# acids-ircam/RAVE

Hardware: NVIDIA H100
Metric: audio-seconds/s (v2 train step fwd+bwd, 48 kHz) (higher is better)
Workload: dtype bf16

## Files before the change

include/rave_b200.h:

```cpp
#ifndef RAVE_B200_H
#define RAVE_B200_H

#include <stddef.h>
#include <stdint.h>

#ifdef __cplusplus
extern "C" {
#endif

#define RAVE_ACT_NONE 0
#define RAVE_ACT_LEAKY 1
#define RAVE_ACT_SNAKE 2

#define RAVE_PREC_FP32 0
#define RAVE_PREC_BF16 1
#define RAVE_PREC_TF32 2

int rave_b200_version(void);
const char *rave_b200_last_error(void);
unsigned long long rave_b200_launch_count(void);

int rave_pqmf_analysis_fwd(const float *x, const float *taps, float *y, int B, int T, int Lout,
                           int ntaps, int pad_l, int flip_sign, void *stream);
int rave_pqmf_synthesis_fwd(const float *x, const float *w, float *out, int B, int L, int K,
                            int pad_l, float scale, int flip_sign, void *stream);
int rave_pqmf_analysis_fast(const float *x, const float *Ct, const float *Qt, float *y, int B, int T, int Lout,
                            int pad_l, int flip_sign, void *stream);
int rave_pqmf_synthesis_fast(const float *x, const float *Cc, const float *Qt, float *out, int B, int L,
                             int pad_l, float scale, int flip_sign, void *stream);

int rave_conv1d_gather_f32(const float *src, const float *w, const float *bias, const float *res,
                           float *out, int B, int Cs, int Ls, int Cm, int Lo, int K, int stride,
                           int dil, int pad_l, long ws_m, long ws_c, int act, float slope,
                           const float *alpha, int post_act, float post_slope, const float *post_x,
                           const float *post_alpha, void *stream);
int rave_conv1d_scatter_f32(const float *src, const float *w, const float *bias, const float *res,
                            float *out, int B, int Cs, int Ls, int Cm, int Lo, int K, int stride,
                            int dil, int pad_l, long ws_m, long ws_c, int act, float slope,
                            const float *alpha, int post_act, float post_slope, const float *post_x,
                            const float *post_alpha, void *stream);

size_t rave_conv1d_wgrad_workspace_bytes(int B, int Ca, int Cc, int Lp, int K);
int rave_conv1d_wgrad_f32(const float *P, const float *Q, float *dw, int B, int Ca, int Lp, int Cc,
                          int Lq, int K, int stride, int dil, int pad_l, long os_a, long os_c,
                          int act_p, int act_q, float slope, const float *alpha, void *workspace,
                          void *stream);

int rave_weight_norm_fwd(const float *v, const float *g, float *w, float *norm_out, int C0, int R,
                         void *stream);
int rave_weight_norm_bwd(const float *dw, const float *v, const float *g, const float *norm,
                         float *dv, float *dg, int C0, int R, void *stream);

int rave_act_fwd(const float *x, float *y, int B, int C, int L, int act, float slope,
                 const float *alpha, void *stream);
int rave_act_bwd(const float *dy, const float *x, float *dx, float *dalpha, int B, int C, int L,
                 int act, float slope, const float *alpha, void *stream);
int rave_am_tanh_fwd(const float *x, float *y, int B, int C, int L, void *stream);
int rave_am_tanh_bwd(const float *dy, const float *x, float *dx, int B, int C, int L, void *stream);
int rave_reparam_fwd(const float *z, const float *eps, float *zs, float *kl_sum, int B, int C, int L, void *stream);
int rave_mmd_fwd(const float *z, const float *prior, float *means, float *mmd, int B, int D, int L, void *stream);
int rave_mmd_bwd(const float *z, const float *prior, const float *g, float *dz, int B, int D, int L, void *stream);
int rave_sphere_norm_fwd(const float *z, float *out, float *norm, int B, int C, int L, void *stream);
int rave_sphere_norm_bwd(const float *g, const float *out, const float *norm, float *dz, int B, int C, int L,
                         void *stream);

int rave_conv1d_tc_supported(int Cin, int Cout, int K, int stride, int dil);
int rave_dilated_unit_tc_supported(int C, int L);
int rave_dilated_unit_tc_fwd(const void *xa_bf16, const void *w3t_bf16, const void *w1t_bf16, void *a1_out,
                             float *out_f32, void *out_act, int B, int C, int L, int pitch, int dil, int pad_l,
                             float slope_in, float slope_mid, int act_out, float slope_out, void *stream);
int rave_conv1d_tc_plan(int B, int Cin, int Cout, int Lout, int K);
int rave_conv1d_tc_pp_stages(int B, int Cin, int Cout, int Lout, int K, int fm, int res_bf16);
int rave_conv1d_tc_fwd(const void *xa_bf16, const void *wt_bf16, const float *bias, const float *res,
                       const void *res_bf16, const void *dact_src_bf16, const void *res_act_bf16, float res_slope,
                       float *out_f32, void *out_act_bf16,
                       int B, int Cin, int Lin, int in_pitch, int Cout, int Lout,
                       int K, int stride, int dil, int pad_l, int act, float slope, int out_rows,
                       int out_row_stride, int out_row_offset, const float *fm_d, int fm_bh, void *stream);
int rave_conv1d_tc_fwd_x3(const void *xa_bf16, const void *wt_bf16, const float *bias, const float *res,
                          const void *res_act, float res_slope, float *out_f32, void *out_act, int B, int Cin, int Lin,
                          int in_pitch, int Cout, int Lout, int K, int stride, int dil, int pad_l, int act, float slope,
                          int out_rows, int out_row_stride, int out_row_offset, int act_cs, void *stream);
int rave_conv1d_tc_wgrad_splits(int B, int Cm, int Lp, int Cn, int K);
int rave_time_stack_cl(const float *x, void *out_bf16, int B, int C, int T, int F, int Fp, int Cp, int kt, int pt,
                       void *stream);
int rave_time_stack_cl_bwd(const void *g_bf16, float *gx, int B, int C, int T, int F, int Fp, int Cp, int kt, int pt,
                           void *stream);
int rave_time_stack_nhwc(const float *x, void *out_bf16, int B, int C, int T, int F, long sb, long st, int Fp, int Cp, int kt,
                         int pt, void *stream);
int rave_time_stack_nhwc_bwd(const void *g_bf16, float *gx, int B, int C, int T, int F, int Fp, int Cp, int kt, int pt,
                             void *stream);
int rave_time_stack_nhwc_dil(const float *x, void *out_bf16, int B, int C, int T, int F, long sb, long st, int Fp, int Cp,
                             int kt, int pt, int dil, void *stream);
int rave_time_stack_nhwc_dil_bwd(const void *g_bf16, float *gx, int B, int C, int T, int F, int Fp, int Cp, int kt, int pt,
                                 int dil, void *stream);
int rave_l1_stats_f32(const float *t, const float *v, float *stats, long n, void *stream);
int rave_l1_grad_f32(const float *t, const float *v, const float *d, float *gt, float *gv, long n, void *stream);
int rave_leaky_fm_fwd(const float *x, float *a, float *stats, long H, float slope, void *stream);
int rave_leaky_fm_bwd(const float *a, const float *g, const float *d, float *gx, long H, float slope, void *stream);
int rave_leaky_fm_stack_fwd(const float *x, float *a, float *stats, void *xs_bf16, long Rh, int T, int F, int C, int Fp,
                            float slope, void *stream);
int rave_leaky_fm_stack_bwd(const float *a, const void *gxs_bf16, const float *ga, const float *d, float *gx, long Rh, int T,
                            int F, int C, int Fp, float slope, void *stream);
int rave_leaky_fm_stack_dil_fwd(const float *x, float *a, float *stats, void *xs_bf16, long Rh, int T, int F, int C, int Fp,
                                int dil, float slope, void *stream);
int rave_leaky_fm_stack_dil_bwd(const float *a, const void *gxs_bf16, const float *ga, const float *d, float *gx, long Rh,
                                int T, int F, int C, int Fp, int dil, float slope, void *stream);
int rave_snake_cl_fwd(const void *h_bf16, const float *alpha, void *a_bf16, long rows, int C, void *stream);
int rave_snake_cl_bwd(const void *ga_bf16, const void *h_bf16, const float *alpha, const void *add_bf16, void *gh_bf16,
                      float *dalpha, long rows, int C, void *stream);
int rave_conv1d_tc_wgrad(const void *P_bf16, const void *Q_bf16, float *dwt, float *dbias, int B, int Cm, int Lp,
                         int p_pitch, int Cn, int Lq, int q_pitch, int K, int stride, int dil, int pad_l,
                         void *stream);
int rave_tapmajor_to_weight_f32(const float *dwt, float *dw, int Cm, int Cn, int K, int transpose, int splits,
                                void *stream);
int rave_conv1d_c1_fwd(const float *x, const float *w, const float *bias, float *out_f32, void *out_act_bf16,
                       int R, int x_pitch, int Lin, int Cout, int Lout, int out_pitch, int K, int stride,
                       int pad_l, int act, float slope, void *stream);
int rave_conv1d_c1_wgrad_splits(int R, int Lout);
int rave_conv1d_c1_wgrad(const void *g_bf16, const float *x, float *dwt, int R, int x_pitch, int Lin, int Cout,
                         int Cg, int Lout, int g_pitch, int K, int stride, int pad_l, void *stream);
int rave_conv1d_c1_dgrad(const void *g_bf16, const float *w, float *dx, int R, int x_pitch, int Lin, int Cout,
                         int Cg, int Lout, int g_pitch, int K, int stride, int pad_l, void *stream);
int rave_colsum_bf16(const void *g_bf16, float *out, int R, int L, int pitch, int Cg, int C, void *stream);
int rave_im2col_c1(const float *src, void *X_bf16, int R, int src_pitch, int src_len, int Lin, int Lout,
// ... 79 lines not shown
```

rave_b200/_lib.py:

```python
import ctypes
import os
from ctypes import c_float, c_int, c_long, c_size_t, c_ulonglong, c_void_p, c_char_p

_HERE = os.path.dirname(os.path.abspath(__file__))
LIB_PATH = os.path.join(_HERE, "csrc", "librave_b200.so")

_P, _I, _F, _L = c_void_p, c_int, c_float, c_long

SIGNATURES = {
    "rave_b200_version": (c_int, []),
    "rave_b200_last_error": (c_char_p, []),
    "rave_b200_launch_count": (c_ulonglong, []),
    "rave_pqmf_analysis_fwd": (c_int, [_P, _P, _P, _I, _I, _I, _I, _I, _I, _P]),
    "rave_pqmf_synthesis_fwd": (c_int, [_P, _P, _P, _I, _I, _I, _I, _F, _I, _P]),
    "rave_pqmf_analysis_fast": (c_int, [_P, _P, _P, _P, _I, _I, _I, _I, _I, _P]),
    "rave_pqmf_synthesis_fast": (c_int, [_P, _P, _P, _P, _I, _I, _I, _F, _I, _P]),
    "rave_conv1d_gather_f32": (c_int, [_P, _P, _P, _P, _P, _I, _I, _I, _I, _I, _I, _I, _I, _I, _L, _L,
                                       _I, _F, _P, _I, _F, _P, _P, _P]),
    "rave_conv1d_scatter_f32": (c_int, [_P, _P, _P, _P, _P, _I, _I, _I, _I, _I, _I, _I, _I, _I, _L, _L,
                                        _I, _F, _P, _I, _F, _P, _P, _P]),
    "rave_conv1d_wgrad_workspace_bytes": (c_size_t, [_I, _I, _I, _I, _I]),
    "rave_conv1d_wgrad_f32": (c_int, [_P, _P, _P, _I, _I, _I, _I, _I, _I, _I, _I, _I, _L, _L, _I, _I,
                                      _F, _P, _P, _P]),
    "rave_weight_norm_fwd": (c_int, [_P, _P, _P, _P, _I, _I, _P]),
    "rave_weight_norm_bwd": (c_int, [_P, _P, _P, _P, _P, _P, _I, _I, _P]),
    "rave_act_fwd": (c_int, [_P, _P, _I, _I, _I, _I, _F, _P, _P]),
    "rave_act_bwd": (c_int, [_P, _P, _P, _P, _I, _I, _I, _I, _F, _P, _P]),
    "rave_am_tanh_fwd": (c_int, [_P, _P, _I, _I, _I, _P]),
    "rave_am_tanh_bwd": (c_int, [_P, _P, _P, _I, _I, _I, _P]),
    "rave_reparam_fwd": (c_int, [_P, _P, _P, _P, _I, _I, _I, _P]),
    "rave_mmd_fwd": (c_int, [_P, _P, _P, _P, _I, _I, _I, _P]),
    "rave_mmd_bwd": (c_int, [_P, _P, _P, _P, _I, _I, _I, _P]),
    "rave_sphere_norm_fwd": (c_int, [_P, _P, _P, _I, _I, _I, _P]),
    "rave_sphere_norm_bwd": (c_int, [_P, _P, _P, _P, _I, _I, _I, _P]),
    "rave_conv1d_tc_supported": (c_int, [_I, _I, _I, _I, _I]),
    "rave_dilated_unit_tc_supported": (c_int, [_I, _I]),
    "rave_dilated_unit_tc_fwd": (c_int, [_P, _P, _P, _P, _P, _P, _I, _I, _I, _I, _I, _I, _F, _F, _I, _F, _P]),
    "rave_conv1d_tc_plan": (c_int, [_I, _I, _I, _I, _I]),
    "rave_conv1d_tc_pp_stages": (c_int, [_I, _I, _I, _I, _I, _I, _I]),
    "rave_conv1d_tc_fwd": (c_int, [_P, _P, _P, _P, _P, _P, _P, _F, _P, _P, _I, _I, _I, _I, _I, _I, _I, _I, _I, _I, _I,
                                   _F, _I, _I, _I, _P, _I, _P]),
    "rave_conv1d_tc_fwd_x3": (c_int, [_P, _P, _P, _P, _P, _F, _P, _P, _I, _I, _I, _I, _I, _I, _I, _I, _I, _I, _I, _F, _I,
                                      _I, _I, _I, _P]),
    "rave_weight_prep_tc_multi_x3": (c_int, [_I, _P, _P]),
    "rave_ncl_to_cl_x3": (c_int, [_P, _P, _I, _I, _I, _P]),
    "rave_conv1d_tc_wgrad": (c_int, [_P, _P, _P, _P, _I, _I, _I, _I, _I, _I, _I, _I, _I, _I, _I, _P]),
    "rave_tapmajor_to_weight_f32": (c_int, [_P, _P, _I, _I, _I, _I, _I, _P]),
    "rave_conv1d_tc_wgrad_splits": (c_int, [_I, _I, _I, _I, _I]),
    "rave_time_stack_cl": (c_int, [_P, _P, _I, _I, _I, _I, _I, _I, _I, _I, _P]),
    "rave_time_stack_cl_bwd": (c_int, [_P, _P, _I, _I, _I, _I, _I, _I, _I, _I, _P]),
    "rave_time_stack_nhwc": (c_int, [_P, _P, _I, _I, _I, _I, ctypes.c_long, ctypes.c_long, _I, _I, _I, _I, _P]),
    "rave_time_stack_nhwc_bwd": (c_int, [_P, _P, _I, _I, _I, _I, _I, _I, _I, _I, _P]),
    "rave_time_stack_nhwc_dil": (c_int, [_P, _P, _I, _I, _I, _I, ctypes.c_long, ctypes.c_long, _I, _I, _I, _I, _I, _P]),
    "rave_time_stack_nhwc_dil_bwd": (c_int, [_P, _P, _I, _I, _I, _I, _I, _I, _I, _I, _I, _P]),
    "rave_l1_stats_f32": (c_int, [_P, _P, _P, ctypes.c_long, _P]),
    "rave_leaky_fm_fwd": (c_int, [_P, _P, _P, ctypes.c_long, ctypes.c_float, _P]),
    "rave_leaky_fm_bwd": (c_int, [_P, _P, _P, _P, ctypes.c_long, ctypes.c_float, _P]),
    "rave_leaky_fm_stack_fwd": (c_int, [_P, _P, _P, _P, ctypes.c_long, _I, _I, _I, _I, ctypes.c_float, _P]),
    "rave_leaky_fm_stack_bwd": (c_int, [_P, _P, _P, _P, _P, ctypes.c_long, _I, _I, _I, _I, ctypes.c_float, _P]),
    "rave_leaky_fm_stack_dil_fwd": (c_int, [_P, _P, _P, _P, ctypes.c_long, _I, _I, _I, _I, _I, ctypes.c_float, _P]),
    "rave_leaky_fm_stack_dil_bwd": (c_int, [_P, _P, _P, _P, _P, ctypes.c_long, _I, _I, _I, _I, _I, ctypes.c_float, _P]),
    "rave_l1_grad_f32": (c_int, [_P, _P, _P, _P, _P, ctypes.c_long, _P]),
    "rave_snake_cl_fwd": (c_int, [_P, _P, _P, ctypes.c_long, _I, _P]),
    "rave_snake_cl_bwd": (c_int, [_P, _P, _P, _P, _P, _P, ctypes.c_long, _I, _P]),
    "rave_weight_prep_tc": (c_int, [_P, _P, _P, _P, _P, _I, _P, _P, _I, _I, _I, _I, _I, _I, _P]),
    "rave_weight_norm_bwd_tapmajor": (c_int, [_P, _P, _P, _P, _P, _P, _I, _I, _I, _I, _I, _I, _P]),
    "rave_conv1d_c1_fwd": (c_int, [_P, _P, _P, _P, _P, _I, _I, _I, _I, _I, _I, _I, _I, _I, _I, _F, _P]),
    "rave_conv1d_c1_wgrad_splits": (c_int, [_I, _I]),
    "rave_conv1d_c1_wgrad": (c_int, [_P, _P, _P, _I, _I, _I, _I, _I, _I, _I, _I, _I, _I, _P]),
    "rave_conv1d_c1_dgrad": (c_int, [_P, _P, _P, _I, _I, _I, _I, _I, _I, _I, _I, _I, _I, _P]),
    "rave_colsum_bf16": (c_int, [_P, _P, _I, _I, _I, _I, _I, _P]),
    "rave_im2col_c1": (c_int, [_P, _P, _I, _I, _I, _I, _I, _I, _I, _I, _I, _I, _I, _P]),
    "rave_gather_c1": (c_int, [_P, _P, _I, _I, _I, _I, _I, _I, _I, _I, _I, _I, _I, _P]),
    "rave_im2col_cin": (c_int, [_P, _P, _I, _I, _I, _I, _I, _I, _I, _I, _I, _I, _I, _I, _I, _P]),
    "rave_gather_cin": (c_int, [_P, _P, _I, _I, _I, _I, _I, _I, _I, _I, _I, _I, _I, _I, _I, _P]),
    "rave_fm_stats": (c_int, [_P, _P, _I, _I, _I, _I, _F, _P]),
    "rave_fm_grad": (c_int, [_P, _P, _P, _I, _I, _I, _I, _F, _P]),
    "rave_score_stats": (c_int, [_P, _P, _I, _I, _I, _I, _P]),
    "rave_score_grad": (c_int, [_P, _P, _P, _I, _I, _I, _I, _P]),
    "rave_spectral_stats": (c_int, [_P, _P, _P, _L, _F, _P]),
    "rave_spectral_grad": (c_int, [_P, _P, _P, _P, _P, _L, _F, _P]),
    "rave_stft_frames": (c_int, [_P, _P, _P, _I, _I, _I, _I, _P]),
    "rave_stft_frames_bwd": (c_int, [_P, _P, _P, _I, _I, _I, _I, _P]),
    "rave_stft_frames_valid": (c_int, [_P, _P, _P, _I, _I, _I, _I, _F, _P]),
    "rave_stft_frames_valid_bwd": (c_int, [_P, _P, _P, _I, _I, _I, _I, _F, _P]),
    "rave_rfft_bwd_scale": (c_int, [_P, _P, _L, _I, _I, _L, _L, _L, _P]),
    "rave_mel_log1p_fwd": (c_int, [_P, _P, _P, _P, _I, _I, _I, _I, _I, _F, _P]),
    "rave_gru_fwd": (c_int, [_P, _P, _P, _P, _P, _I, _I, _I, _P]),
    "rave_gru_bwd": (c_int, [_P, _P, _P, _P, _P, _I, _I, _I, _P]),
    "rave_gemm_f32_splits": (c_int, [_I, _I, _I]),
    "rave_gemm_f32": (c_int, [_P, _L, _L, _P, _L, _L, _P, _P, _L, _P, _I, _I, _I, _P, _I, _P]),
    "rave_noise_fir_fwd": (c_int, [_P, _P, _P, _P, _I, _I, _I, _I, _I, _P]),
# ... 89 lines not shown
```

rave_b200/csrc/conv_tc.cu:

```cuda
#include <string.h>

#include <type_traits>

#include "common.cuh"
#include "tc_common.cuh"

namespace rave {
namespace tc {

constexpr int BLOCK_M = 128;
constexpr int NUM_THREADS = 288;
constexpr int SMEM_MAX = 227 * 1024;

struct TcParams {
  int B, Cin, Lin, Cout, Lout, K, stride, dil, pad_l;
  int BL, BB;
  int n_lt, n_bg, n_nt;
  int num_kb;
  int act;
  float slope;
  const float *bias;
  const float *res;
  const __nv_bfloat16 *res_bf16;
  const __nv_bfloat16 *dact_src;
// ... 369 lines not shown
    float d[2][BLOCK_N / 2];
    int it = 0;
    for (int tile = blockIdx.x; tile < num_tiles; tile += gridDim.x, ++it) {
      const int prev = mma_mainloop<BLOCK_N, BLOCK_K, X3>(d, smem_base, ring, kblocks, lane);
      mma_drain<BLOCK_N>(d, ring, prev, lane);
      const int buf = p.nacc == 2 ? (it & 1) : 0;
      const uint32_t use = p.nacc == 2 ? (it >> 1) : it;
      mbar_wait(&tempty_bar[buf], (use & 1) ^ 1);
      acc_store<BLOCK_N>(d, threadIdx.x, 0, 128 * buf);
      mbar_arrive(&tfull_bar[buf]);
    }
  } else {
    constexpr int BOXC = L::OUT_BOXC;
    const int quad = warp & 3;
    const int row = quad * 32 + lane;
    const bool issuer = threadIdx.x == 160;
    int it = 0;
    for (int tile = blockIdx.x; tile < num_tiles; tile += gridDim.x, ++it) {
      const TileCoord t = tile_coord<BLOCK_N>(tile, p);
      const int n0 = t.n0;
      const int b = t.b0 + row / p.BL;
      const int l = t.l0 + row % p.BL;
      const bool valid = (b < p.B) && (l < p.Lout);
      const size_t orow = (size_t)b * p.out_rows + (size_t)l * p.out_row_stride + p.out_row_offset;

      const int buf = p.nacc == 2 ? (it & 1) : 0;
      const uint32_t use = p.nacc == 2 ? (it >> 1) : it;
      if (stg) {
        if (issuer) bulk_wait_read<0>();
        named_bar_sync(1, 128);
      }
      mbar_wait(&tfull_bar[buf], use & 1);
      const uint32_t taddr = (uint32_t)(128 * buf + quad * 32) << 16;
      tc_epilogue<BLOCK_N, X3, BOXC>(p, taddr, n0, valid, orow, p.fm_d ? (b < p.fm_bh ? 1 : -1) : 0, stg, row);
      __syncwarp();
      if (lane == 0) mbar_arrive(&tempty_bar[buf]);
      if (stg) {
        fence_proxy_async();
        named_bar_sync(1, 128);
        if (issuer) {
#pragma unroll
          for (int c = 0; c < BLOCK_N; c += BOXC)
            tma_store_3d(&tmap_o, stg + (c / BOXC) * (BLOCK_M * L::OUT_SPAN), n0 + c, t.l0, t.b0);
          bulk_commit();
        }
      }
    }
    if (stg && issuer) bulk_wait_all();
  }
}

constexpr int PP_THREADS = 384;

template <int BLOCK_N, int BOXC, bool FM, bool RS>
__device__ __forceinline__ void pp_epilogue(float (*d)[BLOCK_N / 2], uint8_t *slot, const TcParams &p, int w, int lane,
                                            int b0) {
  constexpr int TILE_BYTES = BLOCK_M * BLOCK_N * 2;
  uint8_t *part = slot + TILE_BYTES;
  uint8_t *skip = slot + (FM ? 2 : 1) * TILE_BYTES;
  constexpr int SPAN = BOXC * 2, JB = BOXC / 8;
  const float d0 = FM ? __ldg(p.fm_d) : 0.f, d1 = FM ? __ldg(p.fm_d + 1) : 0.f;
  const uint32_t base = stg_offset<BOXC>(16 * w + (lane >> 2), 0) + 4 * (lane & 3);
#pragma unroll
  for (int h = 0; h < 2; ++h) {
#pragma unroll
    for (int r = 0; r < 2; ++r) {
      const int row = 64 * h + 16 * w + (lane >> 2) + 8 * r;
      const float d1r = (FM && b0 + row / p.BL < p.fm_bh) ? d1 : 0.f;
#pragma unroll
      for (int j = 0; j < BLOCK_N / 8; ++j) {
        const uint32_t off = (base ^ (uint32_t)((j % JB) << 4)) + (j / JB) * (BLOCK_M * SPAN) + (64 * h + 8 * r) * SPAN;
        float v0 = d[h][4 * j + 2 * r], v1 = d[h][4 * j + 2 * r + 1];
        const uint32_t dm = *reinterpret_cast<const uint32_t *>(slot + off);
        lrelu_mask(v0, v1, dm, p.slope);
        if (FM) fm_grad(v0, v1, dm, *reinterpret_cast<const uint32_t *>(part + off), d0, d1r);
        if (RS) add_bf16_pair(v0, v1, *reinterpret_cast<const uint32_t *>(skip + off));
        __nv_bfloat162 o = __floats2bfloat162_rn(v0, v1);
        *reinterpret_cast<uint32_t *>(slot + off) = *reinterpret_cast<uint32_t *>(&o);
      }
    }
  }
}

template <int BLOCK_N, int BLOCK_K, bool FM, bool RS>
__global__ void __launch_bounds__(PP_THREADS, 1)
conv_tc_pp_kernel(const __grid_constant__ CUtensorMap tmap_a, const __grid_constant__ CUtensorMap tmap_b,
                  const __grid_constant__ CUtensorMap tmap_m, const __grid_constant__ CUtensorMap tmap_p,
                  const __grid_constant__ CUtensorMap tmap_r, const __grid_constant__ CUtensorMap tmap_o,
                  const TcParams p) {
  using L = SmemLayout<BLOCK_N, BLOCK_K, false>;
  constexpr int BOXC = L::OUT_BOXC;
  constexpr int BOX_BYTES = BLOCK_M * L::OUT_SPAN;
  constexpr int TILE_BYTES = BLOCK_M * BLOCK_N * 2;
  const int STAGES = p.stages;
  static_assert(BLOCK_N % 16 == 0 && BLOCK_N >= 16 && BLOCK_N <= 128, "invalid wgmma N");

  extern __shared__ uint8_t smem_raw[];
  uint8_t *smem = reinterpret_cast<uint8_t *>((reinterpret_cast<uintptr_t>(smem_raw) + 1023) & ~uintptr_t(1023));
  uint64_t *full_bar = reinterpret_cast<uint64_t *>(smem + p.bar_off);
  uint64_t *empty_bar = full_bar + STAGES;
  uint64_t *ofull_bar = empty_bar + STAGES;
  uint64_t *oempty_bar = ofull_bar + 2;
  uint64_t *order_bar = oempty_bar + 2;

  const int wg = threadIdx.x >> 7;
  const int warp = threadIdx.x >> 5;
  const int lane = threadIdx.x & 31;
  const int num_tiles = p.n_lt * p.n_bg * p.n_nt;
  const int kblocks = p.K * p.num_kb;
  constexpr bool fm = FM, rs = RS;

  if (threadIdx.x == 0) {
    tma_prefetch_desc(&tmap_a);
    tma_prefetch_desc(&tmap_b);
    tma_prefetch_desc(&tmap_m);
    tma_prefetch_desc(&tmap_o);
    if (fm) tma_prefetch_desc(&tmap_p);
    if (rs) tma_prefetch_desc(&tmap_r);
    for (int s = 0; s < STAGES; ++s) {
      mbar_init(&full_bar[s], 1);
      mbar_init(&empty_bar[s], 4);
    }
    for (int c = 0; c < 2; ++c) {
      mbar_init(&ofull_bar[c], 1);
      mbar_init(&oempty_bar[c], 1);
      mbar_init(&order_bar[c], 4);
    }
    fence_barrier_init();
  }
  __syncthreads();
  griddep_launch_dependents();
  griddep_wait();

  if (wg == 0) {
    warpgroup_reg_dealloc<56>();
    if (warp != 0) return;
    Ring ring{full_bar, empty_bar, STAGES, 0, 0};
    int it = 0;
    for (int tile = blockIdx.x; tile < num_tiles; tile += gridDim.x, ++it) {
      const TileCoord t = tile_coord<BLOCK_N>(tile, p);
      const int c = it & 1;
      for (int k = 0; k < p.K; ++k) {
        const TapOrigin o = tap_origin(k, p.dil, p.pad_l, p.stride);
        for (int kb = 0; kb < p.num_kb; ++kb) {
          produce_kblock<BLOCK_N, BLOCK_K, false>(smem, ring, &tmap_a, &tmap_b, p, t, o, k, kb);
          if (k == 0 && kb == 0) {
            mbar_wait(&oempty_bar[c], ((it >> 1) & 1) ^ 1);
            uint8_t *slot = smem + p.ops_off + c * p.ops_bytes;
            if (elect_one()) {
              mbar_arrive_expect_tx(&ofull_bar[c], p.ops_bytes);
              for (int cb = 0; cb < BLOCK_N / BOXC; ++cb) {
                tma_load_3d(slot + cb * BOX_BYTES, &tmap_m, &ofull_bar[c], t.n0 + cb * BOXC, t.l0, t.b0);
                if (fm) {
                  for (int i = 0; i < p.BB; ++i) {
                    const int b = t.b0 + i;
                    const int pb = p.fm_bh > 0 ? (b < p.fm_bh ? b + p.fm_bh : b - p.fm_bh) : b;
                    tma_load_3d(slot + TILE_BYTES + cb * BOX_BYTES + i * p.BL * L::OUT_SPAN, &tmap_p, &ofull_bar[c],
                                t.n0 + cb * BOXC, t.l0, pb);
                  }
                }
                if (rs)
                  tma_load_3d(slot + (fm ? 2 : 1) * TILE_BYTES + cb * BOX_BYTES, &tmap_r, &ofull_bar[c],
                              t.n0 + cb * BOXC, t.l0, t.b0);
              }
            }
            __syncwarp();
          }
        }
      }
    }
  } else {
    warpgroup_reg_alloc<224>();
    const int c = wg - 1;
    const int w = warp & 3;
    const bool issuer = (threadIdx.x & 127) == 0;
    const uint32_t smem_base = smem_u32(smem);
    uint8_t *slot = smem + p.ops_off + c * p.ops_bytes;
    float d[2][BLOCK_N / 2];
    int u = 0;
    for (int tile = blockIdx.x + c * gridDim.x; tile < num_tiles; tile += 2 * gridDim.x, ++u) {
      const int it = 2 * u + c;
      const uint32_t g0 = (uint32_t)it * (uint32_t)kblocks;
      Ring ring{full_bar, empty_bar, STAGES, (int)(g0 % (uint32_t)STAGES), (g0 / (uint32_t)STAGES) & 1};
      if (it > 0) mbar_wait(&order_bar[c], ((it - 1) >> 1) & 1);
      const int prev = mma_mainloop<BLOCK_N, BLOCK_K, false>(d, smem_base, ring, kblocks, lane);
      __syncwarp();
      if (lane == 0) mbar_arrive(&order_bar[c ^ 1]);
      mma_drain<BLOCK_N>(d, ring, prev, lane);

      const TileCoord t = tile_coord<BLOCK_N>(tile, p);
      mbar_wait(&ofull_bar[c], u & 1);
      pp_epilogue<BLOCK_N, BOXC, FM, RS>(d, slot, p, w, lane, t.b0);
      fence_proxy_async();
      named_bar_sync(1 + c, 128);
      if (issuer) {
#pragma unroll
        for (int cb = 0; cb < BLOCK_N / BOXC; ++cb)
          tma_store_3d(&tmap_o, slot + cb * BOX_BYTES, t.n0 + cb * BOXC, t.l0, t.b0);
        bulk_commit();
        bulk_wait_read<0>();
        mbar_arrive(&oempty_bar[c]);
      }
    }
    if (issuer) bulk_wait_all();
  }
}

static CUtensorMapSwizzle swizzle_enum(int bytes) {
  return bytes == 128 ? CU_TENSOR_MAP_SWIZZLE_128B : bytes == 64 ? CU_TENSOR_MAP_SWIZZLE_64B
                                                                 : CU_TENSOR_MAP_SWIZZLE_32B;
}

static int pick_block_k(int Cin) {
  if (Cin % 64 == 0) return 64;
  if (Cin % 32 == 0) return 32;
  if (Cin % 16 == 0) return 16;
  return 0;
}

static int pick_block_n(int Cout, long m_tiles) {
  const int cands[] = {128, 96, 64, 48, 32, 16};
  constexpr int NC = sizeof(cands) / sizeof(cands[0]);
  int best = 0;
  for (int c : cands) {
    if (Cout % c) continue;
    if (!best) best = c;
    if (m_tiles * (Cout / c) >= 132) return c;
  }
  for (int i = NC - 1; i >= 0; --i)
    if (Cout % cands[i] == 0 && cands[i] >= 32) return cands[i];
  return best;
}

struct TcGeometry {
  int BK, BL, BB, n_lt, n_bg, BN, n_nt, num_kb;
};
static TcGeometry tc_geometry(int B, int Cin, int Cout, int Lout) {
  TcGeometry g;
  g.BK = pick_block_k(Cin);
  g.BL = 128;
  while (g.BL > Lout && g.BL > 8) g.BL >>= 1;
  g.BB = 128 / g.BL;
  g.n_lt = ceil_div(Lout, g.BL);
  g.n_bg = ceil_div(B, g.BB);
  g.BN = pick_block_n(Cout, (long)g.n_lt * g.n_bg);
  g.n_nt = g.BN ? Cout / g.BN : 0;
  g.num_kb = g.BK ? ceil_div(Cin, g.BK) : 0;
  return g;
}

template <int BK, typename F>
static int visit_block_n(int BN, F &f) {
  using std::integral_constant;
  switch (BN) {
    case 128: return f(integral_constant<int, BK>(), integral_constant<int, 128>());
    case 96: return f(integral_constant<int, BK>(), integral_constant<int, 96>());
    case 64: return f(integral_constant<int, BK>(), integral_constant<int, 64>());
    case 48: return f(integral_constant<int, BK>(), integral_constant<int, 48>());
    case 32: return f(integral_constant<int, BK>(), integral_constant<int, 32>());
    case 16: return f(integral_constant<int, BK>(), integral_constant<int, 16>());
  }
  set_error("conv1d_tc: no kernel for BLOCK_N=%d", BN);
  return 1;
}
template <typename F>
static int visit_tile(int BK, int BN, F &&f) {
  switch (BK) {
    case 64: return visit_block_n<64>(BN, f);
    case 32: return visit_block_n<32>(BN, f);
    case 16: return visit_block_n<16>(BN, f);
  }
  set_error("conv1d_tc: no kernel for BLOCK_K=%d", BK);
  return 1;
}

template <int BN>
static int encode_rows_map(CUtensorMap *m, const __nv_bfloat16 *base, const TcParams &p, int box_b) {
  using L = SmemLayout<BN, 64, false>;
  const cuuint64_t dims[3] = {(cuuint64_t)p.Cout, (cuuint64_t)p.Lout, (cuuint64_t)p.B};
  const cuuint64_t strides[2] = {(cuuint64_t)p.Cout * 2 * p.out_row_stride, (cuuint64_t)p.Cout * 2 * p.out_rows};
  const cuuint32_t box[3] = {(cuuint32_t)L::OUT_BOXC, (cuuint32_t)p.BL, (cuuint32_t)box_b};
  const CUresult r = encode_bf16_map(m, 3, base + (size_t)p.out_row_offset * p.Cout, dims, strides, box,
                                     swizzle_enum(L::OUT_SPAN), CU_TENSOR_MAP_L2_PROMOTION_NONE);
  if (r != CUDA_SUCCESS) {
    set_error("conv1d_tc: bf16 row tensor map encode failed (%d)", (int)r);
    return 1;
  }
  return 0;
}

template <int BN, int BK>
constexpr bool pp_built = !(BN == 96 && BK == 64);

template <int BN, int BK>
constexpr int pp_stages(int nops) {
  using L = SmemLayout<BN, BK, false>;
  if (!pp_built<BN, BK>) return 0;
  const int s = (SMEM_MAX - L::FIXED - 2 * nops * BLOCK_M * BN * 2) / L::STAGE_BYTES;
  return s < 2 ? 0 : s > 8 ? 8 : s;
}

template <int BN, int BK>
static int launch_pp(const CUtensorMap &ta, const CUtensorMap &tb, TcParams p, int stages, cudaStream_t stream) {
  using L = SmemLayout<BN, BK, false>;
  p.stages = stages;
  p.ops_bytes = (1 + (p.fm_d ? 1 : 0) + (p.res_bf16 ? 1 : 0)) * BLOCK_M * BN * 2;
  p.ops_off = p.stages * L::STAGE_BYTES;
  p.bar_off = p.ops_off + 2 * p.ops_bytes;
  CUtensorMap tm, tp, tr, to;
  memset(&tp, 0, sizeof(tp));
  memset(&tr, 0, sizeof(tr));
  if (encode_rows_map<BN>(&tm, p.dact_src, p, p.BB) || encode_rows_map<BN>(&to, p.out_act, p, p.BB)) return 1;
  if (p.fm_d && encode_rows_map<BN>(&tp, p.fm_bh > 0 ? p.dact_src : p.dact_src - p.fm_half, p, 1)) return 1;
  if (p.res_bf16 && encode_rows_map<BN>(&tr, p.res_bf16, p, p.BB)) return 1;
  const int grid = persistent_grid(p.n_lt * p.n_bg * p.n_nt), smem = p.bar_off + L::FIXED;
  const auto go = [&](auto fm, auto rs) {
    return launch_tc<conv_tc_pp_kernel<BN, BK, decltype(fm)::value, decltype(rs)::value>>(
        "conv1d_tc", grid, PP_THREADS, smem, stream, ta, tb, tm, tp, tr, to, p);
  };
  const std::true_type y;
  const std::false_type n;
  return p.fm_d ? (p.res_bf16 ? go(y, y) : go(y, n)) : (p.res_bf16 ? go(n, y) : go(n, n));
}

template <int BN, int BK, bool X3>
static int launch(const CUtensorMap &ta, const CUtensorMap &tb, TcParams p, cudaStream_t stream) {
  using L = SmemLayout<BN, BK, X3>;
  plan_smem<BN, BK, X3>(p.K * p.num_kb, p);
  if (!p.out_act) p.stg = 0;
  CUtensorMap to;
  memset(&to, 0, sizeof(to));
  if (p.stg && encode_rows_map<BN>(&to, p.out_act, p, p.BB)) return 1;
  return launch_tc<conv_tc_kernel<BN, BK, X3>>("conv1d_tc", persistent_grid(p.n_lt * p.n_bg * p.n_nt), NUM_THREADS,
                                               p.bar_off + L::FIXED, stream, ta, tb, to, p);
}

int conv_tc_dispatch_x3(int BK, int BN, const CUtensorMap &ta, const CUtensorMap &tb, const TcParams &p, cudaStream_t s);
#ifdef RAVE_TC_X3_UNIT
int conv_tc_dispatch_x3(int BK, int BN, const CUtensorMap &ta, const CUtensorMap &tb, const TcParams &p, cudaStream_t s) {
  return visit_tile(BK, BN, [&](auto bk, auto bn) {
    return launch<decltype(bn)::value, decltype(bk)::value, true>(ta, tb, p, s);
  });
}
#endif

}
}

#ifndef RAVE_TC_X3_UNIT
extern "C" int rave_conv1d_tc_supported(int Cin, int Cout, int K, int stride, int dil) {
  if (rave::tc::pick_block_k(Cin) == 0) return 0;
  if (Cout % 16) return 0;
  if (K < 1 || stride < 1 || dil < 1) return 0;
  return 1;
}

extern "C" int rave_conv1d_tc_plan(int B, int Cin, int Cout, int Lout, int K) {
  using namespace rave::tc;
  const TcGeometry g = tc_geometry(B, Cin, Cout, Lout);
  if (!g.BK || !g.BN) return 0;
  TcParams q;
  visit_tile(g.BK, g.BN, [&](auto bk, auto bn) {
    plan_smem<decltype(bn)::value, decltype(bk)::value, false>(K * g.num_kb, q);
    return 0;
  });
  return g.BN | (g.BK << 12) | (q.nacc - 1) << 24 | q.stg << 25 | q.stages << 26;
}

extern "C" int rave_conv1d_tc_pp_stages(int B, int Cin, int Cout, int Lout, int K, int fm, int res_bf16) {
  using namespace rave::tc;
  const TcGeometry g = tc_geometry(B, Cin, Cout, Lout);
  if (!g.BK || !g.BN) return 0;
  const int nops = 1 + (fm ? 1 : 0) + (res_bf16 ? 1 : 0);
  return visit_tile(g.BK, g.BN, [&](auto bk, auto bn) { return pp_stages<decltype(bn)::value, decltype(bk)::value>(nops); });
}

static int conv1d_tc_fwd_impl(const void *xa, const void *wt, const float *bias, const float *res,
                              const void *res_bf16, const void *dact_src, const void *res_act, float res_slope,
                              float *out_f32, void *out_act,
                              int B, int Cin, int Lin, int in_pitch, int Cout, int Lout,
                              int K, int stride, int dil, int pad_l, int act, float slope, int out_rows,
                              int out_row_stride, int out_row_offset, const float *fm_d, int fm_bh,
                              void *stream, int x3, int act_cs = 0) {
  using namespace rave;
  using namespace rave::tc;
  RAVE_CHECK_ARG(!x3 || (!res_bf16 && !dact_src && !fm_d),
                 "conv1d_tc(x3): the split-operand mode has no gradient epilogues (forward path only)");
  RAVE_CHECK_ARG(xa && wt && (out_f32 || out_act), "conv1d_tc: null pointer");
  RAVE_CHECK_ARG(rave_conv1d_tc_supported(Cin, Cout, K, stride, dil), "conv1d_tc: unsupported shape Cin=%d Cout=%d",
                 Cin, Cout);
  if (in_pitch <= 0) in_pitch = Lin;
  RAVE_CHECK_ARG(in_pitch >= ceil_div(Lin, stride) * stride,
                 "conv1d_tc: input pitch %d < Lin %d rounded up to the stride %d (slack rows must be zero)", in_pitch,
                 Lin, stride);
  RAVE_CHECK_ARG(act == RAVE_ACT_NONE || act == RAVE_ACT_LEAKY, "conv1d_tc: epilogue activation %d unsupported", act);
  RAVE_CHECK_ARG(act != RAVE_ACT_LEAKY || (slope >= 0.f && slope <= 1.f), "conv1d_tc: LeakyReLU slope %g outside [0, 1]",
                 (double)slope);
  RAVE_CHECK_ARG(!res_act || (res_slope > 0.f && res_slope <= 1.f), "conv1d_tc: res_slope %g outside (0, 1]",
                 (double)res_slope);
  RAVE_CHECK_ARG(((uintptr_t)bias & 15) == 0, "conv1d_tc: bias must be 16-byte aligned");
  RAVE_CHECK_ARG(((uintptr_t)xa & 15) == 0 && ((uintptr_t)wt & 15) == 0, "conv1d_tc: operands must be 16B aligned");
  RAVE_CHECK_ARG((((uintptr_t)out_f32 | (uintptr_t)out_act | (uintptr_t)res | (uintptr_t)res_bf16 | (uintptr_t)dact_src |
                   (uintptr_t)res_act) & 31) == 0,
                 "conv1d_tc: epilogue tensors must be 32-byte aligned (256-bit row segments)");
  RAVE_CHECK_ARG(get_encode_fn(), "conv1d_tc: cuTensorMapEncodeTiled not available");

  const TcGeometry g = tc_geometry(B, Cin, Cout, Lout);
  RAVE_CHECK_ARG(g.BN > 0, "conv1d_tc: no BLOCK_N for Cout=%d", Cout);
  const int BK = g.BK, BN = g.BN;
  const CUtensorMapL2promotion promo = BK == 64 ? CU_TENSOR_MAP_L2_PROMOTION_L2_256B : CU_TENSOR_MAP_L2_PROMOTION_NONE;
  TcParams p;
  p.B = B; p.Cin = Cin; p.Lin = Lin; p.Cout = Cout; p.Lout = Lout; p.K = K; p.stride = stride; p.dil = dil;
  p.pad_l = pad_l; p.act = act; p.slope = slope; p.bias = bias; p.res = res; p.out_f32 = out_f32;
  p.res_bf16 = (const __nv_bfloat16 *)res_bf16; p.dact_src = (const __nv_bfloat16 *)dact_src;
  p.res_act = (const __nv_bfloat16 *)res_act;
  p.res_inv_slope = (res_act && res_slope > 0.f) ? 1.f / res_slope : 1.f;
  p.out_act = (__nv_bfloat16 *)out_act;
  p.out_rows = out_rows > 0 ? out_rows : Lout;
  p.out_row_stride = out_row_stride > 0 ? out_row_stride : 1;
  p.out_row_offset = out_row_offset;
  RAVE_CHECK_ARG(!fm_d || (dact_src && slope > 0.f && ((fm_bh > 0 && 2 * fm_bh == B) || (fm_bh < 0 && -fm_bh == B))),
                 "conv1d_tc: the fused feature-matching gradient needs dact_src and a [real; fake] batch (B=%d, fm_bh=%d)",
                 B, fm_bh);
  p.fm_d = fm_d;
  p.fm_bh = fm_bh > 0 ? fm_bh : 0;
  p.fm_half = (long)(fm_bh > 0 ? fm_bh : -fm_bh) * p.out_rows * Cout;
  p.act_ld = x3 ? 2 * Cout : Cout;
  p.act_cs = act_cs > 0 ? act_cs : Cout;
  RAVE_CHECK_ARG(!x3 || (Cout % p.act_cs == 0 && p.act_cs % 16 == 0),
                 "conv1d_tc(x3): %d channels per position do not tile the %d-column rows in 16-column chunks", p.act_cs,
                 Cout);
  RAVE_CHECK_ARG(!x3 || !res_act || p.act_cs == Cout, "conv1d_tc(x3): res_act needs one position per row");
  p.BL = g.BL; p.BB = g.BB; p.n_lt = g.n_lt; p.n_bg = g.n_bg; p.n_nt = g.n_nt; p.num_kb = g.num_kb;

  CUtensorMap ta, tb;
  {
    const cuuint64_t ca = (cuuint64_t)Cin * (x3 ? 2 : 1);
    const cuuint64_t dims[4] = {ca, (cuuint64_t)stride, (cuuint64_t)ceil_div(Lin, stride), (cuuint64_t)B};
    const cuuint64_t strides[3] = {ca * 2, ca * 2 * stride, ca * 2 * in_pitch};
    const cuuint32_t box[4] = {(cuuint32_t)BK, 1, (cuuint32_t)p.BL, (cuuint32_t)p.BB};
    const CUresult r = encode_bf16_map(&ta, 4, xa, dims, strides, box, swizzle_enum(BK * 2), promo);
    RAVE_CHECK_ARG(r == CUDA_SUCCESS, "conv1d_tc: tensor map A encode failed (%d)", (int)r);
  }
  {
    const cuuint64_t dims[2] = {(cuuint64_t)Cin, (cuuint64_t)K * Cout * (x3 ? 2 : 1)};
    const cuuint64_t strides[1] = {(cuuint64_t)Cin * 2};
    const cuuint32_t box[2] = {(cuuint32_t)BK, (cuuint32_t)BN};
    const CUresult r = encode_bf16_map(&tb, 2, wt, dims, strides, box, swizzle_enum(BK * 2), promo);
    RAVE_CHECK_ARG(r == CUDA_SUCCESS, "conv1d_tc: tensor map B encode failed (%d)", (int)r);
  }
  cudaStream_t s = (cudaStream_t)stream;
  if (x3) return conv_tc_dispatch_x3(BK, BN, ta, tb, p, s);
  const bool pp = dact_src && out_act && !bias && !res && !res_act && !out_f32 && act == RAVE_ACT_NONE;
  const int nops = 1 + (fm_d ? 1 : 0) + (res_bf16 ? 1 : 0);
  return visit_tile(BK, BN, [&](auto bk, auto bn) {
    constexpr int BK_ = decltype(bk)::value, BN_ = decltype(bn)::value;
    if constexpr (pp_built<BN_, BK_>) {
      const int stages = pp ? pp_stages<BN_, BK_>(nops) : 0;
      if (stages) return launch_pp<BN_, BK_>(ta, tb, p, stages, s);
    }
    return launch<BN_, BK_, false>(ta, tb, p, s);
  });
}

extern "C" int rave_conv1d_tc_fwd(const void *xa, const void *wt, const float *bias, const float *res,
                                  const void *res_bf16, const void *dact_src, const void *res_act, float res_slope,
                                  float *out_f32, void *out_act,
                                  int B, int Cin, int Lin, int in_pitch, int Cout, int Lout,
                                  int K, int stride, int dil, int pad_l, int act, float slope, int out_rows,
                                  int out_row_stride, int out_row_offset, const float *fm_d, int fm_bh,
                                  void *stream) {
  return conv1d_tc_fwd_impl(xa, wt, bias, res, res_bf16, dact_src, res_act, res_slope, out_f32, out_act, B, Cin, Lin,
                            in_pitch, Cout, Lout, K, stride, dil, pad_l, act, slope, out_rows, out_row_stride,
                            out_row_offset, fm_d, fm_bh, stream, 0);
}

extern "C" int rave_conv1d_tc_fwd_x3(const void *xa, const void *wt, const float *bias, const float *res,
                                     const void *res_act, float res_slope, float *out_f32, void *out_act,
                                     int B, int Cin, int Lin, int in_pitch, int Cout, int Lout,
                                     int K, int stride, int dil, int pad_l, int act, float slope, int out_rows,
                                     int out_row_stride, int out_row_offset, int act_cs, void *stream) {
  return conv1d_tc_fwd_impl(xa, wt, bias, res, nullptr, nullptr, res_act, res_slope, out_f32, out_act, B, Cin, Lin,
                            in_pitch, Cout, Lout, K, stride, dil, pad_l, act, slope, out_rows, out_row_stride,
                            out_row_offset, nullptr, 0, stream, 1, act_cs);
}

namespace rave {
namespace tc {

constexpr int WG_ROWS = 64;
constexpr int WG_SLAB = WG_ROWS * 128;

struct WgParams {
  int B, Cm, Lp, Cn, Lq, K, stride, dil, pad_l;
  int BL, BB, n_lt, n_bg;
  int n_mt, n_nt, splits;
  float *dwt;
  float *dbias;
  float *dbias_part;
};

template <int BLOCK_N>
struct WgSmem {
  static constexpr int NS = (BLOCK_N + 63) / 64;
  static constexpr int STAGE_BYTES = (2 + NS) * WG_SLAB;
  static constexpr int MAX_STAGES = (200 * 1024) / STAGE_BYTES;
  static constexpr int STAGES = MAX_STAGES > 6 ? 6 : MAX_STAGES;
  static constexpr int BAR_OFFSET = STAGES * STAGE_BYTES;
  static constexpr int CS_OFFSET = BAR_OFFSET + 256;
  static constexpr int TOTAL = CS_OFFSET + 4096 + 1024;
};

// ... 281 lines not shown
```

Before: 2183.

## Route bf16-only forward convs through the persistent ping-pong TC kernel

Adds a forward variant of the persistent ping-pong tensor-core conv kernel, with a bias/leaky epilogue that writes bf16 through a double-buffered smem slot and TMA store. Forward convs that produce only bf16 activations (no residual or f32 output) now use it when the stage count fits, so the epilogue of one tile overlaps the MMA of the next. The kernel body is shared with the dgrad variant through a compile-time epilogue mask. It costs more template instantiations, and the stage-selection heuristic may pick fewer pipeline stages than the plain kernel would.

```diff
diff --git a/include/rave_b200.h b/include/rave_b200.h
--- a/include/rave_b200.h
+++ b/include/rave_b200.h
@@ -71,6 +71,7 @@
                              float slope_in, float slope_mid, int act_out, float slope_out, void *stream);
 int rave_conv1d_tc_plan(int B, int Cin, int Cout, int Lout, int K);
 int rave_conv1d_tc_pp_stages(int B, int Cin, int Cout, int Lout, int K, int fm, int res_bf16);
+int rave_conv1d_tc_pp_fwd_stages(int B, int Cin, int Cout, int Lout, int K);
 int rave_conv1d_tc_fwd(const void *xa_bf16, const void *wt_bf16, const float *bias, const float *res,
                        const void *res_bf16, const void *dact_src_bf16, const void *res_act_bf16, float res_slope,
                        float *out_f32, void *out_act_bf16,
diff --git a/rave_b200/_lib.py b/rave_b200/_lib.py
--- a/rave_b200/_lib.py
+++ b/rave_b200/_lib.py
@@ -38,6 +38,7 @@
     "rave_dilated_unit_tc_fwd": (c_int, [_P, _P, _P, _P, _P, _P, _I, _I, _I, _I, _I, _I, _F, _F, _I, _F, _P]),
     "rave_conv1d_tc_plan": (c_int, [_I, _I, _I, _I, _I]),
     "rave_conv1d_tc_pp_stages": (c_int, [_I, _I, _I, _I, _I, _I, _I]),
+    "rave_conv1d_tc_pp_fwd_stages": (c_int, [_I, _I, _I, _I, _I]),
     "rave_conv1d_tc_fwd": (c_int, [_P, _P, _P, _P, _P, _P, _P, _F, _P, _P, _I, _I, _I, _I, _I, _I, _I, _I, _I, _I, _I,
                                    _F, _I, _I, _I, _P, _I, _P]),
     "rave_conv1d_tc_fwd_x3": (c_int, [_P, _P, _P, _P, _P, _F, _P, _P, _I, _I, _I, _I, _I, _I, _I, _I, _I, _I, _I, _F, _I,
diff --git a/rave_b200/csrc/conv_tc.cu b/rave_b200/csrc/conv_tc.cu
--- a/rave_b200/csrc/conv_tc.cu
+++ b/rave_b200/csrc/conv_tc.cu
@@ -445,6 +445,8 @@
 
 constexpr int PP_THREADS = 384;
 
+enum PpEpi : int { PP_FM = 1, PP_RS = 2, PP_FWD = 4, PP_BIAS = 8, PP_LEAKY = 16 };
+
 template <int BLOCK_N, int BOXC, bool FM, bool RS>
 __device__ __forceinline__ void pp_epilogue(float (*d)[BLOCK_N / 2], uint8_t *slot, const TcParams &p, int w, int lane,
                                             int b0) {
@@ -475,18 +477,52 @@
   }
 }
 
-template <int BLOCK_N, int BLOCK_K, bool FM, bool RS>
-__global__ void __launch_bounds__(PP_THREADS, 1)
-conv_tc_pp_kernel(const __grid_constant__ CUtensorMap tmap_a, const __grid_constant__ CUtensorMap tmap_b,
-                  const __grid_constant__ CUtensorMap tmap_m, const __grid_constant__ CUtensorMap tmap_p,
-                  const __grid_constant__ CUtensorMap tmap_r, const __grid_constant__ CUtensorMap tmap_o,
-                  const TcParams p) {
+template <int BLOCK_N, int BOXC, bool BIAS, bool LEAKY>
+__device__ __forceinline__ void pp_fwd_epilogue(float (*d)[BLOCK_N / 2], uint8_t *slot, const TcParams &p, int w,
+                                                int lane, int n0) {
+  constexpr int SPAN = BOXC * 2, JB = BOXC / 8;
+  const uint32_t base = stg_offset<BOXC>(16 * w + (lane >> 2), 0) + 4 * (lane & 3);
+  const uint32_t sslot = smem_u32(slot);
+  const float2 *bias = reinterpret_cast<const float2 *>(p.bias + n0 + 2 * (lane & 3));
+#pragma unroll
+  for (int j = 0; j < BLOCK_N / 8; ++j) {
+    const float2 bb = BIAS ? __ldg(bias + 4 * j) : make_float2(0.f, 0.f);
+    const uint32_t col = (base ^ (uint32_t)((j % JB) << 4)) + (j / JB) * (BLOCK_M * SPAN);
+#pragma unroll
+    for (int h = 0; h < 2; ++h) {
+#pragma unroll
+      for (int r = 0; r < 2; ++r) {
+        float v0 = d[h][4 * j + 2 * r], v1 = d[h][4 * j + 2 * r + 1];
+        if (BIAS) {
+          v0 += bb.x;
+          v1 += bb.y;
+        }
+        if (LEAKY) {
+          v0 = fmaxf(v0, v0 * p.slope);
+          v1 = fmaxf(v1, v1 * p.slope);
+        }
+        __nv_bfloat162 o = __floats2bfloat162_rn(v0, v1);
+        asm volatile("st.shared.b32 [%0], %1;" ::"r"(sslot + col + (64 * h + 8 * r) * SPAN),
+                     "r"(*reinterpret_cast<uint32_t *>(&o))
+                     : "memory");
+      }
+    }
+  }
+}
+
+template <int BLOCK_N, int BLOCK_K, int E>
+__device__ __forceinline__ void conv_tc_pp_body(const CUtensorMap *tmap_a, const CUtensorMap *tmap_b,
+                                                const CUtensorMap *tmap_m, const CUtensorMap *tmap_p,
+                                                const CUtensorMap *tmap_r, const CUtensorMap *tmap_o,
+                                                const TcParams &p) {
   using L = SmemLayout<BLOCK_N, BLOCK_K, false>;
   constexpr int BOXC = L::OUT_BOXC;
   constexpr int BOX_BYTES = BLOCK_M * L::OUT_SPAN;
   constexpr int TILE_BYTES = BLOCK_M * BLOCK_N * 2;
+  constexpr bool FWD = E & PP_FWD, FM = E & PP_FM, RS = E & PP_RS;
   const int STAGES = p.stages;
   static_assert(BLOCK_N % 16 == 0 && BLOCK_N >= 16 && BLOCK_N <= 128, "invalid wgmma N");
+  static_assert(!FWD || !(FM || RS), "the forward epilogue has no gradient operands");
 
   extern __shared__ uint8_t smem_raw[];
   uint8_t *smem = reinterpret_cast<uint8_t *>((reinterpret_cast<uintptr_t>(smem_raw) + 1023) & ~uintptr_t(1023));
@@ -501,15 +537,14 @@
   const int lane = threadIdx.x & 31;
   const int num_tiles = p.n_lt * p.n_bg * p.n_nt;
   const int kblocks = p.K * p.num_kb;
-  constexpr bool fm = FM, rs = RS;
 
   if (threadIdx.x == 0) {
-    tma_prefetch_desc(&tmap_a);
-    tma_prefetch_desc(&tmap_b);
-    tma_prefetch_desc(&tmap_m);
-    tma_prefetch_desc(&tmap_o);
-    if (fm) tma_prefetch_desc(&tmap_p);
-    if (rs) tma_prefetch_desc(&tmap_r);
+    tma_prefetch_desc(tmap_a);
+    tma_prefetch_desc(tmap_b);
+    tma_prefetch_desc(tmap_o);
+    if constexpr (!FWD) tma_prefetch_desc(tmap_m);
+    if constexpr (FM) tma_prefetch_desc(tmap_p);
+    if constexpr (RS) tma_prefetch_desc(tmap_r);
     for (int s = 0; s < STAGES; ++s) {
       mbar_init(&full_bar[s], 1);
       mbar_init(&empty_bar[s], 4);
@@ -536,24 +571,24 @@
       for (int k = 0; k < p.K; ++k) {
         const TapOrigin o = tap_origin(k, p.dil, p.pad_l, p.stride);
         for (int kb = 0; kb < p.num_kb; ++kb) {
-          produce_kblock<BLOCK_N, BLOCK_K, false>(smem, ring, &tmap_a, &tmap_b, p, t, o, k, kb);
-          if (k == 0 && kb == 0) {
+          produce_kblock<BLOCK_N, BLOCK_K, false>(smem, ring, tmap_a, tmap_b, p, t, o, k, kb);
+          if (!FWD && k == 0 && kb == 0) {
             mbar_wait(&oempty_bar[c], ((it >> 1) & 1) ^ 1);
             uint8_t *slot = smem + p.ops_off + c * p.ops_bytes;
             if (elect_one()) {
               mbar_arrive_expect_tx(&ofull_bar[c], p.ops_bytes);
               for (int cb = 0; cb < BLOCK_N / BOXC; ++cb) {
-                tma_load_3d(slot + cb * BOX_BYTES, &tmap_m, &ofull_bar[c], t.n0 + cb * BOXC, t.l0, t.b0);
-                if (fm) {
+                tma_load_3d(slot + cb * BOX_BYTES, tmap_m, &ofull_bar[c], t.n0 + cb * BOXC, t.l0, t.b0);
+                if (FM) {
                   for (int i = 0; i < p.BB; ++i) {
                     const int b = t.b0 + i;
                     const int pb = p.fm_bh > 0 ? (b < p.fm_bh ? b + p.fm_bh : b - p.fm_bh) : b;
-                    tma_load_3d(slot + TILE_BYTES + cb * BOX_BYTES + i * p.BL * L::OUT_SPAN, &tmap_p, &ofull_bar[c],
+                    tma_load_3d(slot + TILE_BYTES + cb * BOX_BYTES + i * p.BL * L::OUT_SPAN, tmap_p, &ofull_bar[c],
                                 t.n0 + cb * BOXC, t.l0, pb);
                   }
                 }
-                if (rs)
-                  tma_load_3d(slot + (fm ? 2 : 1) * TILE_BYTES + cb * BOX_BYTES, &tmap_r, &ofull_bar[c],
+                if (RS)
+                  tma_load_3d(slot + (FM ? 2 : 1) * TILE_BYTES + cb * BOX_BYTES, tmap_r, &ofull_bar[c],
                               t.n0 + cb * BOXC, t.l0, t.b0);
               }
             }
@@ -582,14 +617,19 @@
       mma_drain<BLOCK_N>(d, ring, prev, lane);
 
       const TileCoord t = tile_coord<BLOCK_N>(tile, p);
-      mbar_wait(&ofull_bar[c], u & 1);
-      pp_epilogue<BLOCK_N, BOXC, FM, RS>(d, slot, p, w, lane, t.b0);
+      if constexpr (FWD) {
+        mbar_wait(&oempty_bar[c], (u & 1) ^ 1);
+        pp_fwd_epilogue<BLOCK_N, BOXC, (E & PP_BIAS) != 0, (E & PP_LEAKY) != 0>(d, slot, p, w, lane, t.n0);
+      } else {
+        mbar_wait(&ofull_bar[c], u & 1);
+        pp_epilogue<BLOCK_N, BOXC, FM, RS>(d, slot, p, w, lane, t.b0);
+      }
       fence_proxy_async();
       named_bar_sync(1 + c, 128);
       if (issuer) {
 #pragma unroll
         for (int cb = 0; cb < BLOCK_N / BOXC; ++cb)
-          tma_store_3d(&tmap_o, slot + cb * BOX_BYTES, t.n0 + cb * BOXC, t.l0, t.b0);
+          tma_store_3d(tmap_o, slot + cb * BOX_BYTES, t.n0 + cb * BOXC, t.l0, t.b0);
         bulk_commit();
         bulk_wait_read<0>();
         mbar_arrive(&oempty_bar[c]);
@@ -597,6 +637,24 @@
     }
     if (issuer) bulk_wait_all();
   }
+}
+
+template <int BLOCK_N, int BLOCK_K, bool FM, bool RS>
+__global__ void __launch_bounds__(PP_THREADS, 1)
+conv_tc_pp_kernel(const __grid_constant__ CUtensorMap tmap_a, const __grid_constant__ CUtensorMap tmap_b,
+                  const __grid_constant__ CUtensorMap tmap_m, const __grid_constant__ CUtensorMap tmap_p,
+                  const __grid_constant__ CUtensorMap tmap_r, const __grid_constant__ CUtensorMap tmap_o,
+                  const TcParams p) {
+  conv_tc_pp_body<BLOCK_N, BLOCK_K, (FM ? PP_FM : 0) | (RS ? PP_RS : 0)>(&tmap_a, &tmap_b, &tmap_m, &tmap_p, &tmap_r,
+                                                                         &tmap_o, p);
+}
+
+template <int BLOCK_N, int BLOCK_K, bool BIAS, bool LEAKY>
+__global__ void __launch_bounds__(PP_THREADS, 1)
+conv_tc_pp_fwd_kernel(const __grid_constant__ CUtensorMap tmap_a, const __grid_constant__ CUtensorMap tmap_b,
+                      const __grid_constant__ CUtensorMap tmap_o, const TcParams p) {
+  conv_tc_pp_body<BLOCK_N, BLOCK_K, PP_FWD | (BIAS ? PP_BIAS : 0) | (LEAKY ? PP_LEAKY : 0)>(
+      &tmap_a, &tmap_b, nullptr, nullptr, nullptr, &tmap_o, p);
 }
 
 static CUtensorMapSwizzle swizzle_enum(int bytes) {
@@ -682,38 +740,56 @@
   return 0;
 }
 
-template <int BN, int BK>
-constexpr bool pp_built = !(BN == 96 && BK == 64);
-
-template <int BN, int BK>
+template <int BN, int BK, bool FWD>
+constexpr bool pp_built = FWD || !(BN == 96 && BK == 64);
+
+template <int BN, int BK, bool FWD>
 constexpr int pp_stages(int nops) {
   using L = SmemLayout<BN, BK, false>;
-  if (!pp_built<BN, BK>) return 0;
+  if (!pp_built<BN, BK, FWD>) return 0;
   const int s = (SMEM_MAX - L::FIXED - 2 * nops * BLOCK_M * BN * 2) / L::STAGE_BYTES;
   return s < 2 ? 0 : s > 8 ? 8 : s;
 }
 
 template <int BN, int BK>
+static int pp_fwd_stages(int kblocks) {
+  const int s = pp_stages<BN, BK, true>(1);
+  TcParams q;
+  plan_smem<BN, BK, false>(kblocks, q);
+  return s >= q.stages && (BN == 128 || kblocks <= 24) ? s : 0;
+}
+
+template <int BN, int BK, bool FWD>
 static int launch_pp(const CUtensorMap &ta, const CUtensorMap &tb, TcParams p, int stages, cudaStream_t stream) {
   using L = SmemLayout<BN, BK, false>;
   p.stages = stages;
   p.ops_bytes = (1 + (p.fm_d ? 1 : 0) + (p.res_bf16 ? 1 : 0)) * BLOCK_M * BN * 2;
   p.ops_off = p.stages * L::STAGE_BYTES;
   p.bar_off = p.ops_off + 2 * p.ops_bytes;
-  CUtensorMap tm, tp, tr, to;
-  memset(&tp, 0, sizeof(tp));
-  memset(&tr, 0, sizeof(tr));
-  if (encode_rows_map<BN>(&tm, p.dact_src, p, p.BB) || encode_rows_map<BN>(&to, p.out_act, p, p.BB)) return 1;
-  if (p.fm_d && encode_rows_map<BN>(&tp, p.fm_bh > 0 ? p.dact_src : p.dact_src - p.fm_half, p, 1)) return 1;
-  if (p.res_bf16 && encode_rows_map<BN>(&tr, p.res_bf16, p, p.BB)) return 1;
   const int grid = persistent_grid(p.n_lt * p.n_bg * p.n_nt), smem = p.bar_off + L::FIXED;
-  const auto go = [&](auto fm, auto rs) {
-    return launch_tc<conv_tc_pp_kernel<BN, BK, decltype(fm)::value, decltype(rs)::value>>(
-        "conv1d_tc", grid, PP_THREADS, smem, stream, ta, tb, tm, tp, tr, to, p);
-  };
   const std::true_type y;
   const std::false_type n;
-  return p.fm_d ? (p.res_bf16 ? go(y, y) : go(y, n)) : (p.res_bf16 ? go(n, y) : go(n, n));
+  CUtensorMap tm, tp, tr, to;
+  if (encode_rows_map<BN>(&to, p.out_act, p, p.BB)) return 1;
+  if constexpr (FWD) {
+    const auto go = [&](auto bias, auto leaky) {
+      return launch_tc<conv_tc_pp_fwd_kernel<BN, BK, decltype(bias)::value, decltype(leaky)::value>>(
+          "conv1d_tc", grid, PP_THREADS, smem, stream, ta, tb, to, p);
+    };
+    const bool leaky = p.act == RAVE_ACT_LEAKY;
+    return p.bias ? (leaky ? go(y, y) : go(y, n)) : (leaky ? go(n, y) : go(n, n));
+  } else {
+    memset(&tp, 0, sizeof(tp));
+    memset(&tr, 0, sizeof(tr));
+    if (encode_rows_map<BN>(&tm, p.dact_src, p, p.BB)) return 1;
+    if (p.fm_d && encode_rows_map<BN>(&tp, p.fm_bh > 0 ? p.dact_src : p.dact_src - p.fm_half, p, 1)) return 1;
+    if (p.res_bf16 && encode_rows_map<BN>(&tr, p.res_bf16, p, p.BB)) return 1;
+    const auto go = [&](auto fm, auto rs) {
+      return launch_tc<conv_tc_pp_kernel<BN, BK, decltype(fm)::value, decltype(rs)::value>>(
+          "conv1d_tc", grid, PP_THREADS, smem, stream, ta, tb, tm, tp, tr, to, p);
+    };
+    return p.fm_d ? (p.res_bf16 ? go(y, y) : go(y, n)) : (p.res_bf16 ? go(n, y) : go(n, n));
+  }
 }
 
 template <int BN, int BK, bool X3>
@@ -765,7 +841,18 @@
   const TcGeometry g = tc_geometry(B, Cin, Cout, Lout);
   if (!g.BK || !g.BN) return 0;
   const int nops = 1 + (fm ? 1 : 0) + (res_bf16 ? 1 : 0);
-  return visit_tile(g.BK, g.BN, [&](auto bk, auto bn) { return pp_stages<decltype(bn)::value, decltype(bk)::value>(nops); });
+  return visit_tile(g.BK, g.BN, [&](auto bk, auto bn) {
+    return pp_stages<decltype(bn)::value, decltype(bk)::value, false>(nops);
+  });
+}
+
+extern "C" int rave_conv1d_tc_pp_fwd_stages(int B, int Cin, int Cout, int Lout, int K) {
+  using namespace rave::tc;
+  const TcGeometry g = tc_geometry(B, Cin, Cout, Lout);
+  if (!g.BK || !g.BN) return 0;
+  return visit_tile(g.BK, g.BN, [&](auto bk, auto bn) {
+    return pp_fwd_stages<decltype(bn)::value, decltype(bk)::value>(K * g.num_kb);
+  });
 }
 
 static int conv1d_tc_fwd_impl(const void *xa, const void *wt, const float *bias, const float *res,
@@ -844,13 +931,19 @@
   }
   cudaStream_t s = (cudaStream_t)stream;
   if (x3) return conv_tc_dispatch_x3(BK, BN, ta, tb, p, s);
-  const bool pp = dact_src && out_act && !bias && !res && !res_act && !out_f32 && act == RAVE_ACT_NONE;
+  const bool bf16_only = out_act && !res && !res_act && !out_f32;
+  const bool pp_dgrad = bf16_only && dact_src && !bias && act == RAVE_ACT_NONE;
+  const bool pp_fwd = bf16_only && !dact_src && !res_bf16 && !fm_d;
   const int nops = 1 + (fm_d ? 1 : 0) + (res_bf16 ? 1 : 0);
   return visit_tile(BK, BN, [&](auto bk, auto bn) {
     constexpr int BK_ = decltype(bk)::value, BN_ = decltype(bn)::value;
-    if constexpr (pp_built<BN_, BK_>) {
-      const int stages = pp ? pp_stages<BN_, BK_>(nops) : 0;
-      if (stages) return launch_pp<BN_, BK_>(ta, tb, p, stages, s);
+    if constexpr (pp_built<BN_, BK_, false>) {
+      const int stages = pp_dgrad ? pp_stages<BN_, BK_, false>(nops) : 0;
+      if (stages) return launch_pp<BN_, BK_, false>(ta, tb, p, stages, s);
+    }
+    if constexpr (pp_built<BN_, BK_, true>) {
+      const int stages = pp_fwd ? pp_fwd_stages<BN_, BK_>(K * g.num_kb) : 0;
+      if (stages) return launch_pp<BN_, BK_, true>(ta, tb, p, stages, s);
     }
     return launch<BN_, BK_, false>(ta, tb, p, s);
   });
```

New measurement: 2282, median of 6. +4.6%, better.
